# Peterande/SAST

Hardware: AMD Instinct MI355X
Metric: frames/sec (B=4) SAST backbone fwd+bwd, 1Mpx 640x360 (higher is better)
Workload: dtype f32; 1 GPU; 1Mpx 640x360 (padded 384x640) full SAST backbone + PAFPN, fwd+bwd + AdamW, B=4/GPU, binary events (rand>0.5), random-init, AMP=0.0002; global_batch=4, seq_len=1, parallelism=dp1, hipgraph=True, library=sast_amd/libsast_hip.so, product_library=True, segmented_backward_overlap=False, deferred_weight_gradients=False, backward_cuts=3, dw_discard_TIMING_PROBE_gradients_invalid=False, collective_ranks=1, collective_ranks_verified=1, gradient_bytes_per_rank=67663616, sync_batchnorm=False, event_dtype=int32, grads_finite=True

## Files before the change

### sast_amd/csrc/gemm.cuh

```cuda
#pragma once
#include <type_traits>
#include <hip/hip_ext.h>
#include "common.cuh"
#include "../../include/sast_hip.h"

#if defined(SAST_TL_ENABLE) && !defined(SAST_TL)
static __device__ unsigned long long sast_tl_buf[8 * 8192];
#define SAST_TL(k)                                                                                          \
  do {                                                                                                      \
    const unsigned bid_ = blockIdx.x;                                                                       \
    if (threadIdx.x == 0 && bid_ < 8192) sast_tl_buf[bid_ * 8 + (k)] = wall_clock64();                      \
    if (threadIdx.x == 0 && bid_ < 8192 && (k) == 0) sast_tl_buf[bid_ * 8 + 7] = __smid();                 \
  } while (0)
#define SAST_TL_JOB(j) do { if (threadIdx.x == 0 && blockIdx.x < 8192) sast_tl_buf[blockIdx.x * 8 + 6] = (j); } while (0)
#endif
#ifndef SAST_TL
#define SAST_TL(k)
#endif
#ifndef SAST_TL_JOB
#define SAST_TL_JOB(j)
#endif
#ifndef SAST_TLF
#define SAST_TLF_DECL
#define SAST_TLF(k)
// ... 118 lines not shown
template <class L, class = void> struct LoaderExactBf16 : std::false_type {};
template <class L> struct LoaderExactBf16<L, std::void_t<decltype(L::EXACT_BF16)>> : std::bool_constant<L::EXACT_BF16> {};
template <class L, class = void> struct LoaderExactAlways : std::false_type {};
template <class L> struct LoaderExactAlways<L, std::void_t<decltype(L::EXACT_BF16_ALWAYS)>> : std::bool_constant<L::EXACT_BF16_ALWAYS> {};
template <class EP, class = void> struct EpHasStats : std::false_type {};
template <class EP> struct EpHasStats<EP, std::void_t<decltype(EP::COLSTATS)>> : std::bool_constant<EP::COLSTATS> {};

using buf_rsrc = __amdgpu_buffer_rsrc_t;
constexpr unsigned BUF_INVALID = 0x80000000u;
constexpr unsigned BUF_MAX_BYTES = 0x80000000u;
__device__ __forceinline__ buf_rsrc make_buf(const void* p, unsigned bytes) {
  const unsigned long long a = reinterpret_cast<unsigned long long>(p);
  const unsigned lo = __builtin_amdgcn_readfirstlane((unsigned)a), hi = __builtin_amdgcn_readfirstlane((unsigned)(a >> 32));
  return __builtin_amdgcn_make_buffer_rsrc(reinterpret_cast<void*>(((unsigned long long)hi << 32) | lo), 0,
                                           __builtin_amdgcn_readfirstlane(bytes), 0x00020000);
}
__device__ __forceinline__ float4 ldb(buf_rsrc d, unsigned off) {
  return __builtin_bit_cast(float4, __builtin_amdgcn_raw_buffer_load_b128(d, off, 0, 0));
}
__device__ __forceinline__ float ldb1(buf_rsrc d, unsigned off) {
  return __uint_as_float(__builtin_amdgcn_raw_buffer_load_b32(d, off, 0, 0));
}
struct BufDesc { buf_rsrc d; };
template <class L, class = void> struct LoaderBuffered : std::false_type {};
template <class L> struct LoaderBuffered<L, std::void_t<decltype(L::BUFFERED)>> : std::bool_constant<L::BUFFERED> {};
struct NoDesc {};
template <class L> __device__ __forceinline__ auto loader_desc(const L& l, int Rl) {
  if constexpr (LoaderBuffered<L>::value) return l.desc(Rl); else return NoDesc{};
}
constexpr unsigned long long BUF_SPAN_LIMIT = 0x80000000ull;
constexpr int BUF_SPAN_SLACK_ROWS = 64;
template <class L> inline bool loader_span_ok(const L& l, int I, int G, int R) {
  if constexpr (LoaderBuffered<L>::value) return l.span_bytes(I, G, R) < BUF_SPAN_LIMIT; else return true;
}

template <class T, class L>
struct OperandPresplitWanted { static constexpr bool value = SAST_MFMA_SPLIT3 && !SAST_MFMA_BF16 && L::RC && (T::BK == 16 || T::BK == 32) && T::KS <= 4 && T::G < 3; };
constexpr int PS_ROW_FLOATS = 3 * 16 / 2;
__device__ __forceinline__ constexpr int ps_chunk_swizzle(int row) { return (row >> 3) & 1; }
constexpr int PS_MAX_FLOATS = 20480;
template <class T, class L, int W>
struct OperandPresplitIC {
  static constexpr bool value = SAST_MFMA_SPLIT3 && !SAST_MFMA_BF16 && !L::RC && (T::BK == 16 || T::BK == 32) && T::KS <= 4 && T::G < 3 &&
                                (W == 32 || W == 64 || W == 128);
};
template <int W> __device__ __forceinline__ constexpr int psi_swizzle(int k) { return W == 64 ? ((k >> 1) & 1) << 3 : W == 128 ? (k & 3) << 3 : 0; }
// ... 152 lines not shown
    for (int it = 0; it < A_PER; ++it)
      if (A_SLOTS % NT == 0 || tid + it * NT < A_SLOTS) {
        const float4 v = la.finish(ra[set][it], aa[set][it], oa[set][it]);
        if constexpr (SPLIT && !LA::RC) {
          if (do_colsum) { csacc[it].x += v.x; csacc[it].y += v.y; csacc[it].z += v.z; csacc[it].w += v.w; }
        }
        if constexpr (PSA && EA) store_hi(as + la_off[it], v);
        else if constexpr (PSA) store_split3(as + la_off[it], BM * 8, v);
        else st4(as + la_off[it], v);
      }
#pragma unroll
    for (int it = 0; it < B_PER; ++it)
      if (B_SLOTS % NT == 0 || tid + it * NT < B_SLOTS) {
        if constexpr (PSB && EB) store_hi(bs + lb_off[it], lb.finish(rb[set][it], ab[set][it], ob[set][it]));
        else if constexpr (PSB) store_split3(bs + lb_off[it], BN * 8, lb.finish(rb[set][it], ab[set][it], ob[set][it]));
        else st4(bs + lb_off[it], lb.finish(rb[set][it], ab[set][it], ob[set][it]));
      }
  };

  typename EP::Col ecol[T::TJ];
#pragma unroll
  for (int tj = 0; tj < T::TJ; ++tj) ecol[tj] = ep.col(min(j0 + (wn * T::TJ + tj) * 32 + (lane & 31), NJ - 1));
  constexpr bool EARLY_AUX = T::TM * T::TJ == 1;
  typename EP::Aux eaux[EARLY_AUX ? 16 : 1];

  f32x16 acc[T::TM][T::TN];
#pragma unroll
  for (int a = 0; a < T::TM; ++a)
#pragma unroll
    for (int b = 0; b < T::TN; ++b)
#pragma unroll
      for (int e = 0; e < 16; ++e) acc[a][b][e] = 0.f;
  float csum[T::TM];
#pragma unroll
  for (int a = 0; a < T::TM; ++a) csum[a] = 0.f;

  auto compute = [&](int buf, auto ex) {
    constexpr bool EA = decltype(ex)::value && XA, EB = decltype(ex)::value && XB;
    const float* as = As + buf * A_STAGE;
    const float* bs = Bs + buf * B_STAGE;
    const int l31 = lane & 31, hf = lane >> 5;
    if constexpr (SAST_MFMA_SPLIT3 && !SAST_MFMA_BF16 && PSA && PSB) {
#pragma unroll
      for (int u = 0; u < BK / 16; ++u) {
        Split3 sa[T::TM], sb[T::TN];
#pragma unroll
// ... 238 lines not shown
#pragma unroll
      for (int a = 0; a < T::TM; ++a)
#pragma unroll
        for (int b = 0; b < T::TN; ++b)
#pragma unroll
          for (int e = 0; e < 16; ++e) acc[a][b][e] += src[((a * T::TN + b) * 16 + e) * 64];
    }
  }

  if (SPLIT && LA::RC && do_colsum) {
#pragma unroll
    for (int t = 0; t < T::TM; ++t) {
      const float s = csum[t] + __shfl_xor(csum[t], 32, 64);
      const int m = m0 + wm * T::WTM + t * 32 + (lane & 31);
      if (lane < 32 && m < Meff) atomicAdd(colsum + m, s);
    }
  }

  SAST_TL(3);
  constexpr bool STATS = EpHasStats<EP>::value;
  float cs[T::TJ], cq[T::TJ];
#pragma unroll
  for (int tj = 0; tj < T::TJ; ++tj) { cs[tj] = 0.f; cq[tj] = 0.f; }
  auto emit = [&](auto inside) {
    constexpr bool INSIDE = decltype(inside)::value;
#pragma unroll
    for (int ta = 0; ta < T::TM; ++ta)
#pragma unroll
      for (int tj = 0; tj < T::TJ; ++tj) {
        const int j = j0 + (wn * T::TJ + tj) * 32 + (lane & 31);
        const int jc = INSIDE ? j : min(j, NJ - 1);
        const int mb = m0 + wm * T::WTM + ta * 32 + 4 * (lane >> 5);
        const typename EP::Col col = ecol[tj];
        typename EP::Aux aux[16];
#pragma unroll
        for (int reg = 0; reg < 16; ++reg) {
          if constexpr (EARLY_AUX) aux[reg] = eaux[reg];
          else aux[reg] = ep.pre(INSIDE ? mb + (reg & 3) + 8 * (reg >> 2) : min(mb + (reg & 3) + 8 * (reg >> 2), Meff - 1), jc);
        }
#pragma unroll
        for (int reg = 0; reg < 16; ++reg) {
          const int m = mb + (reg & 3) + 8 * (reg >> 2);
          if (INSIDE || (m < Meff && j < NJ)) {
            float v[G];
#pragma unroll
            for (int g = 0; g < G; ++g) v[g] = acc[ta][tj * G + g][reg];
            ep.post(m, j, v, col, aux[reg]);
            if constexpr (STATS) ep.stat(v[0], col, aux[reg], cs[tj], cq[tj]);
          }
        }
      }
  };
  if (m0 + BM <= Meff && j0 + BJ <= NJ) emit(std::true_type{});
  else emit(std::false_type{});
  if constexpr (STATS) {
#pragma unroll
    for (int tj = 0; tj < T::TJ; ++tj) {
      const float s = cs[tj] + __shfl_xor(cs[tj], 32, 64), q = cq[tj] + __shfl_xor(cq[tj], 32, 64);
      const int j = j0 + (wn * T::TJ + tj) * 32 + (lane & 31);
      if (lane < 32 && j < NJ) ep.flush(((m0 / BM) * T::WAVES_M + wm) % BN_STAT_COPIES, j, NJ, s, q);
    }
  }
  SAST_TL(4);
}

template <class T, class LA, class LB, class EP, bool SPLIT>
__global__ __launch_bounds__(T::NT, T::MINW) void gemm_kernel(LA la, LB lb, EP ep, int M, int NJ, int R,
                                                              const int* __restrict__ dM, const int* __restrict__ dR,
                                                              float* __restrict__ colsum, int nsplit, int xcd_remap) {
  __shared__ __attribute__((aligned(16))) float smem[GemmSmem<T, LA, LB>::FLOATS];
  kernarg_warm<(int)(sizeof(LA) + sizeof(LB) + sizeof(EP) + 3 * sizeof(int) + 3 * sizeof(void*) + 2 * sizeof(int))>();
  int nmain = gridDim.x;
  if constexpr (EpHasSide<EP>::value) {
    nmain -= ep.side_blocks;
    if ((int)blockIdx.x >= nmain) { ep.side(blockIdx.x - nmain); return; }
  }
  gemm_body<T, LA, LB, EP, SPLIT>(la, lb, ep, M, NJ, R, dM, dR, colsum, nsplit, xcd_remap, blockIdx.x, nmain, smem);
// ... 37 lines not shown
  static double get(const L& l) { return l.src_bytes(); }
};
void prof_kernel_events_ex(const char* tag, double flops, double bytes, hipStream_t st, hipEvent_t* e0, hipEvent_t* e1);
void prof_sum_k(const int* Kw, int W, hipStream_t st, double* sum_k, double* sum_k2);
bool prof_enabled();
void prof_flops_credit(double flops);
bool xcd_remap_enabled();
void prof_scope(const char* name, int c, int m, hipStream_t st, bool begin);
struct ProfScope {
  const char* n; int c, m; hipStream_t st; bool on;
  ProfScope(const char* n_, int c_, int m_, hipStream_t s_) : n(n_), c(c_), m(m_), st(s_), on(prof_enabled()) { if (on) prof_scope(n, c, m, st, true); }
  ~ProfScope() { if (on) prof_scope(n, c, m, st, false); }
};

template <class T, class LA, class LB>
inline bool gemm_span_ok(const LA& la, const LB& lb, int M, int NJ, int R) {
  return loader_span_ok(la, M, 1, R) && loader_span_ok(lb, NJ, T::G, R);
}

template <class T, class LA, class LB, class EP>
inline int launch_gemm(const LA& la, const LB& lb, const EP& ep, int M, int NJ, int R, const int* dM,
                       const int* dR, hipStream_t st) {
  if (M <= 0 || NJ <= 0 || R <= 0) return SAST_OK;
  if (!gemm_span_ok<T>(la, lb, M, NJ, R)) return SAST_EINVAL;
  const int nb = ((M + T::BM - 1) / T::BM) * ((NJ + T::BJ - 1) / T::BJ);
  const int remap = xcd_remap_enabled() && nb >= 16;
  const int grid = remap ? (nb + 7) / 8 * 8 : nb;
  if (prof_enabled()) {
    hipEvent_t e0, e1;
    prof_kernel_events(__PRETTY_FUNCTION__, T::G, M, NJ, R, dM, dR, st, &e0, &e1, LoaderSrcBytes<LA>::get(la), LoaderSrcBytes<LB>::get(lb));
    SAST_EXT_LAUNCH((gemm_kernel<T, LA, LB, EP, false>), dim3(grid + ep_side_blocks(ep)), dim3(T::NT), 0, st, e0, e1, 0, la, lb, ep, M, NJ,
                          R, dM, dR, (float*)nullptr, 1, remap);
  } else {
    SAST_LAUNCH((gemm_kernel<T, LA, LB, EP, false>), dim3(grid + ep_side_blocks(ep)), dim3(T::NT), 0, st, la, lb, ep, M, NJ, R, dM, dR,
                       (float*)nullptr, 1, remap);
  }
  SAST_CHECK_LAUNCH();
  return SAST_OK;
}

template <class T, class LA, class LB, class EP>
inline int launch_gemm_split(const LA& la, const LB& lb, const EP& ep, int M, int NJ, int R, const int* dR,
                             int splits, float* colsum, hipStream_t st) {
  if (M <= 0 || NJ <= 0 || R <= 0) return SAST_OK;
  if (colsum != nullptr && LA::RC && GemmSmem<T, LA, LB>::PSA) return SAST_EINVAL;
  if (!gemm_span_ok<T>(la, lb, M, NJ, R)) return SAST_EINVAL;
  const int nb = ((M + T::BM - 1) / T::BM) * ((NJ + T::BJ - 1) / T::BJ);
  if (splits < 1) splits = 1;
  const int remap = xcd_remap_enabled() && nb * splits >= 16;
  const int grid = remap ? (nb * splits + 7) / 8 * 8 : nb * splits;
  if (prof_enabled()) {
    hipEvent_t e0, e1;
    prof_kernel_events(__PRETTY_FUNCTION__, T::G, M, NJ, R, nullptr, dR, st, &e0, &e1, LoaderSrcBytes<LA>::get(la), LoaderSrcBytes<LB>::get(lb));
    SAST_EXT_LAUNCH((gemm_kernel<T, LA, LB, EP, true>), dim3(grid), dim3(T::NT), 0, st, e0, e1, 0, la, lb, ep, M, NJ, R,
                          (const int*)nullptr, dR, colsum, splits, remap);
  } else {
    SAST_LAUNCH((gemm_kernel<T, LA, LB, EP, true>), dim3(grid), dim3(T::NT), 0, st, la, lb, ep, M, NJ, R,
                       (const int*)nullptr, dR, colsum, splits, remap);
  }
  SAST_CHECK_LAUNCH();
  return SAST_OK;
}

inline int gemm_grid(int ntile, int nsplit, int& remap) {
  const int n = ntile * nsplit;
  remap = xcd_remap_enabled() && n >= 16;
  return remap ? (n + 7) / 8 * 8 : n;
}
void prof_kernel_events2(const char* tag, double flops_static, int G1, int M1, int NJ1, int R1, const int* dM1, const int* dR1, int G2,
                         int M2, int NJ2, int R2, const int* dM2, const int* dR2, hipStream_t st, hipEvent_t* e0, hipEvent_t* e1,
                         double a1_cap = -1.0, double b1_cap = -1.0, double a2_cap = -1.0, double b2_cap = -1.0);

template <class TS, class LA1, class LB1, class EP1, class TP, class LA2, class LB2, class EP2>
inline int launch_gemm_dual(const LA1& la1, const LB1& lb1, const EP1& ep1, int M1, int NJ1, int R1, const int* dR1, int splits,
                            float* colsum, const LA2& la2, const LB2& lb2, const EP2& ep2, int M2, int NJ2, int R2, const int* dM2,
                            hipStream_t st) {
  using J1 = GemmJob<TS, LA1, LB1, EP1, true>;
  using J2 = GemmJob<TP, LA2, LB2, EP2, false>;
  if (colsum != nullptr && LA1::RC && GemmSmem<TS, LA1, LB1>::PSA) return SAST_EINVAL;
  if (!gemm_span_ok<TS>(la1, lb1, M1, NJ1, R1) || !gemm_span_ok<TP>(la2, lb2, M2, NJ2, R2)) return SAST_EINVAL;
  if (splits < 1) splits = 1;
  const int nt1 = ((M1 + TS::BM - 1) / TS::BM) * ((NJ1 + TS::BJ - 1) / TS::BJ);
  const int nt2 = ((M2 + TP::BM - 1) / TP::BM) * ((NJ2 + TP::BJ - 1) / TP::BJ);
  int r1, r2;
  int n1 = gemm_grid(nt1, splits, r1);
  const int n2 = gemm_grid(nt2, 1, r2);
  if (r2 && (n1 & 7)) n1 = (n1 + 7) / 8 * 8;
  const J1 a{la1, lb1, ep1, M1, NJ1, R1, nullptr, dR1, colsum, splits, r1};
  const J2 b{la2, lb2, ep2, M2, NJ2, R2, dM2, nullptr, nullptr, 1, r2};
  constexpr int NTHREADS = TS::NT > TP::NT ? TS::NT : TP::NT;
  if (prof_enabled()) {
    hipEvent_t e0, e1;
    prof_kernel_events2(__PRETTY_FUNCTION__, 0.0, TS::G, M1, NJ1, R1, nullptr, dR1, TP::G, M2, NJ2, R2, dM2, nullptr, st, &e0, &e1,
                        LoaderSrcBytes<LA1>::get(la1), LoaderSrcBytes<LB1>::get(lb1), LoaderSrcBytes<LA2>::get(la2), LoaderSrcBytes<LB2>::get(lb2));
    SAST_EXT_LAUNCH((gemm_dual_kernel<J1, J2>), dim3(n1 + n2 + ep_side_blocks(ep2)), dim3(NTHREADS), 0, st, e0, e1, 0, a, b, n1);
  } else {
    SAST_LAUNCH((gemm_dual_kernel<J1, J2>), dim3(n1 + n2 + ep_side_blocks(ep2)), dim3(NTHREADS), 0, st, a, b, n1);
  }
  SAST_CHECK_LAUNCH();
  return SAST_OK;
}

using TileBig   = Tile<128, 128, 2, 2, 1>;
// ... 501 lines not shown
    return c;
  }
  __device__ __forceinline__ int reduce_len(int m0) const { return k.slots(m0 / k.Mc) * Cout; }
  __device__ __forceinline__ void load(const Desc& d, const Ctx& c, int r0, int off, int Rl, int, float4& v, float& aux, bool& ok) const {
    const int r = r0 + off, rr = min(r, Rl - 1);
    const int slot = (int)__umulhi((unsigned)rr, cout_mul), co = rr - slot * Cout;
    const int kh = (c.kh >> (4 * slot)) & 15, kw = (c.kw >> (4 * slot)) & 15;
    const bool empty = kh == 15 || kw == 15;
    ok = (r < Rl) & !empty;
    v = ldb(d.d, ok ? c.col + 4u * (unsigned)((co * taps + (empty ? 0 : kh * KW + kw)) * Cin) : BUF_INVALID);
    aux = 0.f;
  }
  SAST_DEFAULT_FINISH
};

inline int pow2_shift(int v) {
  int s = 0;
  while ((1 << s) < v) ++s;
  return (1 << s) == v ? s : -1;
}

struct EpNone {};
struct EpStore {
  float* c; int ldc; const float* bias;
  struct Col { float b; };
  using Aux = EpNone;
  __device__ __forceinline__ Col col(int j) const { return Col{bias ? bias[j] : 0.f}; }
  __device__ __forceinline__ Aux pre(int, int) const { return Aux{}; }
  __device__ __forceinline__ void post(int m, int j, const float (&v)[1], const Col& k, const Aux&) const {
    c[(size_t)m * ldc + j] = v[0] + k.b;
  }
};
struct EpStoreStats {
  static constexpr bool COLSTATS = true;
  float* c; int ldc; double* sums;
  using Col = EpNone; using Aux = EpNone;
  __device__ __forceinline__ Col col(int) const { return Col{}; }
  __device__ __forceinline__ Aux pre(int, int) const { return Aux{}; }
  __device__ __forceinline__ void post(int m, int j, const float (&v)[1], const Col&, const Aux&) const { c[(size_t)m * ldc + j] = v[0]; }
  __device__ __forceinline__ void stat(float v, const Col&, const Aux&, float& a, float& b) const { a += v; b += v * v; }
  __device__ __forceinline__ void flush(int copy, int j, int NJ, float s, float q) const {
    double* sp = sums + (size_t)copy * 2 * NJ;
    atomicAdd(sp + j, (double)s); atomicAdd(sp + NJ + j, (double)q);
  }
};

struct BnProducer {
  const float* x;
  const float* stats;
  const float* gamma; const float* beta;
  float* sums;
  int C;
};
struct BnCol { float mu, rs, g, b; };
__device__ __forceinline__ BnCol bn_col(const BnProducer& p, int j) { return BnCol{p.stats[j], p.stats[p.C + j], p.gamma[j], p.beta[j]}; }
__device__ __forceinline__ void bn_stat(float dy, float x, const BnCol& k, float& a, float& b) {
  const float xh = (x - k.mu) * k.rs;
  const float z = xh * k.g + k.b, sg = sigmoid_hw(z);
  const float dz = dy * sg * (1.f + z * (1.f - sg));
  a += dz; b += dz * xh;
}
struct EpStoreBnRed {
  static constexpr bool COLSTATS = true;
  float* c; int ldc; BnProducer p;
  using Col = BnCol;
  struct Aux { float x; };
  __device__ __forceinline__ Col col(int j) const { return bn_col(p, j); }
  __device__ __forceinline__ Aux pre(int m, int j) const { return Aux{p.x[(size_t)m * p.C + j]}; }
  __device__ __forceinline__ void post(int m, int j, const float (&v)[1], const Col&, const Aux&) const { c[(size_t)m * ldc + j] = v[0]; }
  __device__ __forceinline__ void stat(float v, const Col& k, const Aux& x, float& a, float& b) const { bn_stat(v, x.x, k, a, b); }
  __device__ __forceinline__ void flush(int copy, int j, int, float s, float q) const {
    float* sp = p.sums + (size_t)copy * 2 * p.C;
    atomicAdd(sp + j, s); atomicAdd(sp + p.C + j, q);
  }
};
struct EpStoreAdd {
  float* c; int ldc; const float* add; int ldadd;
  using Col = EpNone;
  struct Aux { float a; };
  __device__ __forceinline__ Col col(int) const { return Col{}; }
  __device__ __forceinline__ Aux pre(int m, int j) const { return Aux{add[(size_t)m * ldadd + j]}; }
  __device__ __forceinline__ void post(int m, int j, const float (&v)[1], const Col&, const Aux& x) const {
    c[(size_t)m * ldc + j] = v[0] + x.a;
  }
};
struct EpStoreStats2 {
  static constexpr bool COLSTATS = true;
  float* c1; float* c2; int C; double* sums1; double* sums2;
  using Col = EpNone; using Aux = EpNone;
  __device__ __forceinline__ Col col(int) const { return Col{}; }
  __device__ __forceinline__ Aux pre(int, int) const { return Aux{}; }
  __device__ __forceinline__ void post(int m, int j, const float (&v)[1], const Col&, const Aux&) const {
    if (j < C) c1[(size_t)m * C + j] = v[0];
    else c2[(size_t)m * C + (j - C)] = v[0];
  }
  __device__ __forceinline__ void stat(float v, const Col&, const Aux&, float& a, float& b) const { a += v; b += v * v; }
  __device__ __forceinline__ void flush(int copy, int j, int, float s, float q) const {
    double* sp = (j < C ? sums1 : sums2) + (size_t)copy * 2 * C;
    const int jj = j < C ? j : j - C;
    atomicAdd(sp + jj, (double)s); atomicAdd(sp + C + jj, (double)q);
  }
};
struct EpAtomic2 {
  float* c1; float* c2; int ldc; int M1;
  using Col = EpNone; using Aux = EpNone;
  __device__ __forceinline__ Col col(int) const { return Col{}; }
  __device__ __forceinline__ Aux pre(int, int) const { return Aux{}; }
  __device__ __forceinline__ void post(int m, int j, const float (&v)[1], const Col&, const Aux&) const {
    atomicAdd((m < M1 ? c1 + (size_t)m * ldc : c2 + (size_t)(m - M1) * ldc) + j, v[0]);
  }
};
struct EpAtomic {
  float* c; int ldc;
  using Col = EpNone; using Aux = EpNone;
  __device__ __forceinline__ Col col(int) const { return Col{}; }
  __device__ __forceinline__ Aux pre(int, int) const { return Aux{}; }
  __device__ __forceinline__ void post(int m, int j, const float (&v)[1], const Col&, const Aux&) const {
    atomicAdd(c + (size_t)m * ldc + j, v[0]);
  }
};

struct EpStoreClass {
  float* c; int ldc; int H, W; ConvDxClasses k;
  using Col = EpNone;
  struct Aux { int p; };
  __device__ __forceinline__ Col col(int) const { return Col{}; }
  __device__ __forceinline__ Aux pre(int m, int) const {
    const int cls = fast_div(m, k.Mc, k.mc_mul), ic = m - cls * k.Mc;
    const int t = fast_div(ic, k.Wc, k.wc_mul), xx = ic - t * k.Wc, b = fast_div(t, k.Hc, k.hc_mul), yy = t - b * k.Hc;
    const int q = 3 - cls;
    return Aux{(b * H + 2 * yy + (q >> 1)) * W + 2 * xx + (q & 1)};
  }
  __device__ __forceinline__ void post(int, int j, const float (&v)[1], const Col&, const Aux& a) const {
    c[(size_t)a.p * ldc + j] = v[0];
  }
};

struct EpSplit2BnRed {
  static constexpr bool COLSTATS = true;
  float* a; float* b; int C1, C2; BnProducer pa, pb;
  using Col = BnCol;
  struct Aux { float x; };
  __device__ __forceinline__ Col col(int j) const {
    if (j < C1) return pa.x ? bn_col(pa, j) : BnCol{0.f, 0.f, 0.f, 0.f};
    return pb.x ? bn_col(pb, j - C1) : BnCol{0.f, 0.f, 0.f, 0.f};
  }
  __device__ __forceinline__ Aux pre(int m, int j) const {
    if (j < C1) return Aux{pa.x ? pa.x[(size_t)m * C1 + j] : 0.f};
    return Aux{pb.x ? pb.x[(size_t)m * C2 + (j - C1)] : 0.f};
  }
  __device__ __forceinline__ void post(int m, int j, const float (&v)[1], const Col&, const Aux&) const {
    if (j < C1) a[(size_t)m * C1 + j] = v[0];
    else if (b) b[(size_t)m * C2 + (j - C1)] = v[0];
  }
  __device__ __forceinline__ void stat(float v, const Col& k, const Aux& x, float& s, float& q) const { bn_stat(v, x.x, k, s, q); }
  __device__ __forceinline__ void flush(int copy, int j, int, float s, float q) const {
    if (j < C1) {
      if (pa.x) { float* sp = pa.sums + (size_t)copy * 2 * C1; atomicAdd(sp + j, s); atomicAdd(sp + C1 + j, q); }
    } else if (pb.x) {
      float* sp = pb.sums + (size_t)copy * 2 * C2; atomicAdd(sp + (j - C1), s); atomicAdd(sp + C2 + (j - C1), q);
    }
  }
};

struct EpSplit2 {
  float* a; float* b; int C1, C2;
  using Col = EpNone; using Aux = EpNone;
  __device__ __forceinline__ Col col(int) const { return Col{}; }
  __device__ __forceinline__ Aux pre(int, int) const { return Aux{}; }
  __device__ __forceinline__ void post(int m, int j, const float (&v)[1], const Col&, const Aux&) const {
    if (j < C1) a[(size_t)m * C1 + j] = v[0];
    else if (b) b[(size_t)m * C2 + (j - C1)] = v[0];
  }
};

}
```

### sast_amd/csrc/gemm_kloop.inc

```
#pragma unroll
  for (int u = 0; u < PF; ++u) gload(tile_of(u), u);
  lstore(0, 0, ex);
  group_sync();
  SAST_TL(1);
  int i = 0;
  SAST_TLF_DECL
  for (; i + PF <= n_it; i += PF) {
#pragma unroll
    for (int u = 0; u < PF; ++u) {
      gload(tile_of(i + u + PF), u);
      SAST_PHASE_FENCE();
      SAST_TLF(0);
      compute(u & 1, ex);
      SAST_TLF(1);
      SAST_TLF_WAIT_OLDER(A_PER + B_PER);
      lstore((u + 1) & 1, (u + 1) % PF, ex);
      SAST_TLF(2);
      group_sync();
      SAST_TLF(3);
      SAST_TLF_COUNT();
    }
  }
  SAST_TLF_FLUSH();
  if constexpr (EARLY_AUX) {
    const int jc = min(j0 + wn * 32 + (lane & 31), NJ - 1), mb = m0 + wm * T::WTM + 4 * (lane >> 5);
#pragma unroll
    for (int reg = 0; reg < 16; ++reg) eaux[reg] = ep.pre(min(mb + (reg & 3) + 8 * (reg >> 2), Meff - 1), jc);
  }
  {
    const int rem = n_it - i;
#pragma unroll
    for (int u = 0; u < PF - 1; ++u) {
      if (u < rem) {
        compute(u & 1, ex);
        lstore((u + 1) & 1, (u + 1) % PF, ex);
        group_sync();
      }
    }
  }
```

### sast_amd/csrc/k_block.hip

```cpp
#include <cstdlib>
#include "gemm_dispatch.cuh"
#include "kernels.h"

using namespace sast;

namespace {

constexpr int ATTN_MAX_T = 256;

struct EpBiasRelu {
  float* c; int ldc; const float* bias;
  struct Col { float b; };
  using Aux = EpNone;
  __device__ __forceinline__ Col col(int j) const { return Col{bias[j]}; }
  __device__ __forceinline__ Aux pre(int, int) const { return Aux{}; }
  __device__ __forceinline__ void post(int m, int j, const float (&v)[1], const Col& k, const Aux&) const {
    c[(size_t)m * ldc + j] = fmaxf(v[0] + k.b, 0.f);
  }
};
struct EpBiasReluCtl : EpBiasRelu {
  static constexpr bool SIDE = true;
  ControlsJob k; int side_blocks;
  __device__ __forceinline__ void side(int sb) const { if (threadIdx.x < 256) controls_fwd_elem(k, sb * 256 + threadIdx.x); }
};
struct EpStoreAddCtl : EpStoreAdd {
  static constexpr bool SIDE = true;
  ControlsJob k; int side_blocks;
  __device__ __forceinline__ void side(int sb) const { if (threadIdx.x < 256) controls_bwd_elem(k, sb * 256 + threadIdx.x); }
};
template <bool RS>
struct EpResidualLST {
  float* y; const float* res; const float* bias; const float* gamma; int C; const float* rs;
  struct Col { float b, g; };
  struct Aux { float r, d; };
  __device__ __forceinline__ Col col(int j) const { return Col{bias[j], gamma ? gamma[j] : 1.f}; }
  __device__ __forceinline__ Aux pre(int m, int j) const { return Aux{res[(size_t)m * C + j], RS ? rs[m] : 1.f}; }
  __device__ __forceinline__ void post(int m, int j, const float (&v)[1], const Col& k, const Aux& x) const {
    if constexpr (RS) y[(size_t)m * C + j] = x.r + (k.g * (v[0] + k.b)) * x.d;
    else y[(size_t)m * C + j] = x.r + k.g * (v[0] + k.b);
  }
};
template <bool RS>
struct EpResidualLSScatterT {
  float* out; const float* res; const float* bias; const float* gamma; const int* row_tok; int C; const float* rs;
  struct Col { float b, g; };
  struct Aux { float r, d; int row; };
  __device__ __forceinline__ Col col(int j) const { return Col{bias[j], gamma ? gamma[j] : 1.f}; }
  __device__ __forceinline__ Aux pre(int m, int j) const { return Aux{res[(size_t)m * C + j], RS ? rs[m] : 1.f, row_tok[m]}; }
  __device__ __forceinline__ void post(int, int j, const float (&v)[1], const Col& k, const Aux& x) const {
    if constexpr (RS) out[(size_t)x.row * C + j] = x.r + (k.g * (v[0] + k.b)) * x.d;
    else out[(size_t)x.row * C + j] = x.r + k.g * (v[0] + k.b);
  }
};
constexpr int PRELU_SLOTS = 1024;
__global__ void __launch_bounds__(PRELU_SLOTS) prelu_slope_finish_kernel(const float* __restrict__ slots, float* __restrict__ d) {
  __shared__ float s[PRELU_SLOTS];
  s[threadIdx.x] = slots[threadIdx.x];
  __syncthreads();
  for (int o = PRELU_SLOTS / 2; o; o >>= 1) {
    if ((int)threadIdx.x < o) s[threadIdx.x] += s[threadIdx.x + o];
    __syncthreads();
  }
  if (threadIdx.x == 0) d[0] += s[0];
}
template <bool ANY>
struct EpGluT {
  float* ug; float* h; const float* bias; int inner; int act;
  const float* drop;
  const float* act_w;
  struct Col { float bu, bg, a; };
  using Aux = EpNone;
  __device__ __forceinline__ Col col(int j) const { return Col{bias[j], bias[inner + j], (ANY && act_w) ? act_w[0] : 0.0f}; }
  __device__ __forceinline__ Aux pre(int, int) const { return Aux{}; }
  __device__ __forceinline__ void post(int m, int j, const float (&v)[2], const Col& k, const Aux&) const {
    const float u = v[0] + k.bu, g = v[1] + k.bg;
    float* ugm = ug + (size_t)m * 2 * inner;
    ugm[j] = u;
    (ugm + inner)[j] = g;
    if constexpr (ANY) h[(size_t)m * inner + j] = (u * glu_act(g, act, k.a)) * (drop ? drop[(size_t)m * inner + j] : 1.f);
    else h[(size_t)m * inner + j] = u * gelu_erf(g);
  }
};
template <bool ANY>
struct EpDGluT {
  const float* ug; float* dug; int inner; int act;
  const float* drop;
  const float* act_w;
  float* slope_slots;
  struct Col { float a; };
  struct Aux { float u, g; };
  __device__ __forceinline__ Col col(int) const { return Col{(ANY && act_w) ? act_w[0] : 0.0f}; }
  __device__ __forceinline__ Aux pre(int m, int j) const { return Aux{ug[(size_t)m * 2 * inner + j], ug[(size_t)m * 2 * inner + inner + j]}; }
  __device__ __forceinline__ void post(int m, int j, const float (&v)[1], const Col& k, const Aux& x) const {
    if constexpr (ANY) {
      const float dh = drop ? v[0] * drop[(size_t)m * inner + j] : v[0];
      dug[(size_t)m * 2 * inner + j] = dh * glu_act(x.g, act, k.a);
      dug[(size_t)m * 2 * inner + inner + j] = dh * x.u * glu_act_grad(x.g, act, k.a);
      if (slope_slots && x.g < 0.0f) atomicAdd(slope_slots + (((size_t)m * inner + j) & (PRELU_SLOTS - 1)), dh * x.u * x.g);
    } else {
      dug[(size_t)m * 2 * inner + j] = v[0] * gelu_erf(x.g);
      dug[(size_t)m * 2 * inner + inner + j] = v[0] * x.u * gelu_erf_grad(x.g);
    }
  }
};
struct EpAddGather {
  float* c; int ldc; const float* src; const int* idx; int lds;
  using Col = EpNone;
  struct Aux { float a; };
  __device__ __forceinline__ Col col(int) const { return Col{}; }
  __device__ __forceinline__ Aux pre(int m, int j) const { return Aux{src[(size_t)idx[m] * lds + j]}; }
  __device__ __forceinline__ void post(int m, int j, const float (&v)[1], const Col&, const Aux& x) const {
    c[(size_t)m * ldc + j] = v[0] + x.a;
  }
};
struct EpLstm {
  const float* bias; const float* c0; float* h1; float* c1; float* gates; int C;
  const float* drop;
  struct Col { float bf, bi, bo, bg; };
  struct Aux { float c, d; };
  __device__ __forceinline__ Col col(int j) const { return Col{bias[j], bias[C + j], bias[2 * C + j], bias[3 * C + j]}; }
  __device__ __forceinline__ Aux pre(int m, int j) const { return Aux{c0 ? c0[(size_t)m * C + j] : 0.f, drop ? drop[(size_t)m * C + j] : 1.f}; }
  __device__ __forceinline__ void post(int m, int j, const float (&v)[4], const Col& k, const Aux& x) const {
    const float f = sigmoid_hw(v[0] + k.bf), i = sigmoid_hw(v[1] + k.bi);
    const float o = sigmoid_hw(v[2] + k.bo), g = tanh_hw(v[3] + k.bg);
    const float c = f * x.c + i * (g * x.d);
    c1[(size_t)m * C + j] = c;
    h1[(size_t)m * C + j] = o * tanh_hw(c);
    float* gp = gates + (size_t)m * 4 * C + j;
    gp[0] = f; gp[C] = i; gp[2 * C] = o; gp[3 * C] = g;
  }
};
struct EpLstm3 {
  const float* bias; float* h1; float* c1; float* gates; int C; const float* drop;
  struct Col { float bi, bo, bg; };
  struct Aux { float d; };
  __device__ __forceinline__ Col col(int j) const { return Col{bias[C + j], bias[2 * C + j], bias[3 * C + j]}; }
  __device__ __forceinline__ Aux pre(int m, int j) const { return Aux{drop ? drop[(size_t)m * C + j] : 1.f}; }
  __device__ __forceinline__ void post(int m, int j, const float (&v)[3], const Col& k, const Aux& x) const {
    const float i = sigmoid_hw(v[0] + k.bi), o = sigmoid_hw(v[1] + k.bo), g = tanh_hw(v[2] + k.bg);
    const float c = 0.f + i * (g * x.d);
    c1[(size_t)m * C + j] = c;
    h1[(size_t)m * C + j] = o * tanh_hw(c);
    float* gp = gates + (size_t)m * 4 * C + j;
    gp[C] = i; gp[2 * C] = o; gp[3 * C] = g;
  }
};
inline bool lstm_skip_f(const SastLstmArgs* a) { return !a->c0 && SAST_KNOB("SAST_LSTM_SKIP_DEAD_GATE", 1) != 0; }

template <bool SKIPF>
__global__ __launch_bounds__(256) void lstm_bwd_pointwise_kernel(const float* __restrict__ gates, const float* __restrict__ c0,
                                                                 const float* __restrict__ c1, const float* __restrict__ dh1,
                                                                 const float* __restrict__ dh1b, const float* __restrict__ dc1,
                                                                 float* __restrict__ dmix,
                                                                 float* __restrict__ dc0, size_t n, int C, unsigned c_mul,
                                                                 const float* __restrict__ drop) {
  const size_t e = (size_t)blockIdx.x * 256 + threadIdx.x;
  if (e >= n) return;
  const size_t m = fast_div((int)e, C, c_mul); const int j = (int)(e - m * C);
  const float* gp = gates + m * 4 * C + j;
  const float f = SKIPF ? 0.f : gp[0], i = gp[C], o = gp[2 * C], g = gp[3 * C];
  const float tc = tanh_hw(c1[e]);
  const float dh = dh1[e] + (dh1b ? dh1b[e] : 0.f);
  const float dc = (dc1 ? dc1[e] : 0.f) + dh * o * (1.f - tc * tc);
  const float cp = (!SKIPF && c0) ? c0[e] : 0.f;
  float* dp = dmix + m * 4 * C + j;
  if constexpr (!SKIPF) dp[0] = dc * cp * f * (1.f - f);
  const float d = drop ? drop[e] : 1.f;
// ... 390 lines not shown
```

Before: 888.5 frames/s.

## Use buffer-resource stores and loads in GEMM epilogues with hardware OOB masking

Adds a buffered epilogue path in which each epilogue builds AMDGPU buffer descriptors for its output and aux tensors and does every store and aux load through raw buffer ops. Offsets are 32-bit with wave-uniform bases, and out-of-range rows and columns are dropped by the descriptor bound or an invalid offset instead of per-element branches and clamping. This aims to cut 64-bit address arithmetic and branch overhead in the epilogue. The cost is span checks that reject tensors above 2GB and extra logic for split-output epilogues where a tile straddles the boundary between the two outputs.

New measurement: 895.0 frames/s (median of 6 runs). About the same (+0.7%).

```diff
diff --git a/sast_amd/csrc/gemm.cuh b/sast_amd/csrc/gemm.cuh
--- a/sast_amd/csrc/gemm.cuh
+++ b/sast_amd/csrc/gemm.cuh
@@ -164,6 +164,34 @@
   return __uint_as_float(__builtin_amdgcn_raw_buffer_load_b32(d, off, 0, 0));
 }
 struct BufDesc { buf_rsrc d; };
+__device__ __forceinline__ buf_rsrc out_buf(const void* p, int Meff, int ld) {
+  return make_buf(p, p ? 4u * (unsigned)Meff * (unsigned)ld : 0u);
+}
+__device__ __forceinline__ void stb(buf_rsrc d, unsigned off, float v) {
+  __builtin_amdgcn_raw_buffer_store_b32(__float_as_uint(v), d, off, 0, 0);
+}
+struct EpAt {
+  int m, j;
+  unsigned lane_col;
+  unsigned lane_rows;
+  int mu;
+  int jt;
+  __device__ __forceinline__ unsigned at(int ld, int dj = 0) const {
+    return (lane_col + 4u * (lane_rows * (unsigned)ld + (unsigned)dj)) + 4u * (unsigned)(mu * ld);
+  }
+};
+struct EpSide { bool right, straddle; };
+__device__ __forceinline__ EpSide ep_side(const EpAt& e, int C1) { return EpSide{e.jt + 32 > C1, e.jt < C1 && e.jt + 32 > C1}; }
+__device__ __forceinline__ EpAt ep_mask(EpAt e, bool keep) { e.lane_col = keep ? e.lane_col : BUF_INVALID; return e; }
+template <class EP, class = void> struct EpBuffered : std::false_type {};
+template <class EP> struct EpBuffered<EP, std::void_t<decltype(EP::BUFFERED)>> : std::bool_constant<EP::BUFFERED> {};
+constexpr int EP_SPAN_SLACK_ROWS = 128;
+inline bool ep_span(int M, int ld, int cols) {
+  return 4ull * ((unsigned long long)(M + EP_SPAN_SLACK_ROWS) * (unsigned long long)ld + (unsigned long long)cols) < 0x80000000ull;
+}
+template <class EP> inline bool ep_span_ok(const EP& ep, int M, int NJ) {
+  if constexpr (EpBuffered<EP>::value) return ep.span_ok(M, NJ); else return true;
+}
 template <class L, class = void> struct LoaderBuffered : std::false_type {};
 template <class L> struct LoaderBuffered<L, std::void_t<decltype(L::BUFFERED)>> : std::bool_constant<L::BUFFERED> {};
 struct NoDesc {};
@@ -362,6 +390,14 @@
 #pragma unroll
   for (int tj = 0; tj < T::TJ; ++tj) ecol[tj] = ep.col(min(j0 + (wn * T::TJ + tj) * 32 + (lane & 31), NJ - 1));
   constexpr bool EARLY_AUX = T::TM * T::TJ == 1;
+  struct EpBase { int mu0, jt0; };
+  auto ep_base = [&]() { return EpBase{__builtin_amdgcn_readfirstlane(m0 + wm * T::WTM), __builtin_amdgcn_readfirstlane(j0 + wn * T::TJ * 32)}; };
+  auto ep_at = [&](const EpBase& eb, int ta, int tj, int reg) {
+    const int j = j0 + (wn * T::TJ + tj) * 32 + (lane & 31);
+    const int mu = eb.mu0 + ta * 32 + (reg & 3) + 8 * (reg >> 2);
+    const unsigned lr = 4u * (unsigned)(lane >> 5);
+    return EpAt{mu + (int)lr, j, j < NJ ? 4u * (unsigned)j : BUF_INVALID, lr, mu, eb.jt0 + tj * 32};
+  };
   typename EP::Aux eaux[EARLY_AUX ? 16 : 1];
 
   f32x16 acc[T::TM][T::TN];
@@ -646,7 +682,7 @@
   float cs[T::TJ], cq[T::TJ];
 #pragma unroll
   for (int tj = 0; tj < T::TJ; ++tj) { cs[tj] = 0.f; cq[tj] = 0.f; }
-  auto emit = [&](auto inside) {
+  auto emit = [&](auto inside, const auto& epx) {
     constexpr bool INSIDE = decltype(inside)::value;
 #pragma unroll
     for (int ta = 0; ta < T::TM; ++ta)
@@ -660,7 +696,7 @@
 #pragma unroll
         for (int reg = 0; reg < 16; ++reg) {
           if constexpr (EARLY_AUX) aux[reg] = eaux[reg];
-          else aux[reg] = ep.pre(INSIDE ? mb + (reg & 3) + 8 * (reg >> 2) : min(mb + (reg & 3) + 8 * (reg >> 2), Meff - 1), jc);
+          else aux[reg] = epx.pre(INSIDE ? mb + (reg & 3) + 8 * (reg >> 2) : min(mb + (reg & 3) + 8 * (reg >> 2), Meff - 1), jc);
         }
 #pragma unroll
         for (int reg = 0; reg < 16; ++reg) {
@@ -669,14 +705,39 @@
             float v[G];
 #pragma unroll
             for (int g = 0; g < G; ++g) v[g] = acc[ta][tj * G + g][reg];
-            ep.post(m, j, v, col, aux[reg]);
-            if constexpr (STATS) ep.stat(v[0], col, aux[reg], cs[tj], cq[tj]);
+            epx.post(m, j, v, col, aux[reg]);
+            if constexpr (STATS) epx.stat(v[0], col, aux[reg], cs[tj], cq[tj]);
           }
         }
       }
   };
-  if (m0 + BM <= Meff && j0 + BJ <= NJ) emit(std::true_type{});
-  else emit(std::false_type{});
+  if constexpr (EpBuffered<EP>::value) {
+    const auto edesc = ep.desc(Meff);
+    const EpBase eb = ep_base();
+#pragma unroll
+    for (int ta = 0; ta < T::TM; ++ta)
+#pragma unroll
+      for (int tj = 0; tj < T::TJ; ++tj) {
+        const typename EP::Col col = ecol[tj];
+        typename EP::Aux aux[16];
+#pragma unroll
+        for (int reg = 0; reg < 16; ++reg) {
+          if constexpr (EARLY_AUX) aux[reg] = eaux[reg];
+          else aux[reg] = ep.pre(edesc, ep_at(eb, ta, tj, reg));
+        }
+#pragma unroll
+        for (int reg = 0; reg < 16; ++reg) {
+          float v[G];
+#pragma unroll
+          for (int g = 0; g < G; ++g) v[g] = acc[ta][tj * G + g][reg];
+          ep.post(edesc, ep_at(eb, ta, tj, reg), v, col, aux[reg]);
+          if constexpr (STATS) ep.stat(v[0], col, aux[reg], cs[tj], cq[tj]);
+        }
+      }
+  } else {
+    if (m0 + BM <= Meff && j0 + BJ <= NJ) emit(std::true_type{}, ep);
+    else emit(std::false_type{}, ep);
+  }
   if constexpr (STATS) {
 #pragma unroll
     for (int tj = 0; tj < T::TJ; ++tj) {
@@ -760,7 +821,7 @@
 inline int launch_gemm(const LA& la, const LB& lb, const EP& ep, int M, int NJ, int R, const int* dM,
                        const int* dR, hipStream_t st) {
   if (M <= 0 || NJ <= 0 || R <= 0) return SAST_OK;
-  if (!gemm_span_ok<T>(la, lb, M, NJ, R)) return SAST_EINVAL;
+  if (!gemm_span_ok<T>(la, lb, M, NJ, R) || !ep_span_ok(ep, M, NJ)) return SAST_EINVAL;
   const int nb = ((M + T::BM - 1) / T::BM) * ((NJ + T::BJ - 1) / T::BJ);
   const int remap = xcd_remap_enabled() && nb >= 16;
   const int grid = remap ? (nb + 7) / 8 * 8 : nb;
@@ -782,7 +843,7 @@
                              int splits, float* colsum, hipStream_t st) {
   if (M <= 0 || NJ <= 0 || R <= 0) return SAST_OK;
   if (colsum != nullptr && LA::RC && GemmSmem<T, LA, LB>::PSA) return SAST_EINVAL;
-  if (!gemm_span_ok<T>(la, lb, M, NJ, R)) return SAST_EINVAL;
+  if (!gemm_span_ok<T>(la, lb, M, NJ, R) || !ep_span_ok(ep, M, NJ)) return SAST_EINVAL;
   const int nb = ((M + T::BM - 1) / T::BM) * ((NJ + T::BJ - 1) / T::BJ);
   if (splits < 1) splits = 1;
   const int remap = xcd_remap_enabled() && nb * splits >= 16;
@@ -817,6 +878,7 @@
   using J2 = GemmJob<TP, LA2, LB2, EP2, false>;
   if (colsum != nullptr && LA1::RC && GemmSmem<TS, LA1, LB1>::PSA) return SAST_EINVAL;
   if (!gemm_span_ok<TS>(la1, lb1, M1, NJ1, R1) || !gemm_span_ok<TP>(la2, lb2, M2, NJ2, R2)) return SAST_EINVAL;
+  if (!ep_span_ok(ep1, M1, NJ1) || !ep_span_ok(ep2, M2, NJ2)) return SAST_EINVAL;
   if (splits < 1) splits = 1;
   const int nt1 = ((M1 + TS::BM - 1) / TS::BM) * ((NJ1 + TS::BJ - 1) / TS::BJ);
   const int nt2 = ((M2 + TP::BM - 1) / TP::BM) * ((NJ2 + TP::BJ - 1) / TP::BJ);
@@ -1364,22 +1426,29 @@
 
 struct EpNone {};
 struct EpStore {
+  static constexpr bool BUFFERED = true;
   float* c; int ldc; const float* bias;
   struct Col { float b; };
   using Aux = EpNone;
+  struct Desc { buf_rsrc c; };
+  bool span_ok(int M, int NJ) const { return ep_span(M, ldc, NJ); }
+  __device__ __forceinline__ Desc desc(int Meff) const { return Desc{out_buf(c, Meff, ldc)}; }
   __device__ __forceinline__ Col col(int j) const { return Col{bias ? bias[j] : 0.f}; }
-  __device__ __forceinline__ Aux pre(int, int) const { return Aux{}; }
-  __device__ __forceinline__ void post(int m, int j, const float (&v)[1], const Col& k, const Aux&) const {
-    c[(size_t)m * ldc + j] = v[0] + k.b;
+  __device__ __forceinline__ Aux pre(const Desc&, const EpAt&) const { return Aux{}; }
+  __device__ __forceinline__ void post(const Desc& d, const EpAt& e, const float (&v)[1], const Col& k, const Aux&) const {
+    stb(d.c, e.at(ldc), v[0] + k.b);
   }
 };
 struct EpStoreStats {
-  static constexpr bool COLSTATS = true;
+  static constexpr bool COLSTATS = true, BUFFERED = true;
   float* c; int ldc; double* sums;
   using Col = EpNone; using Aux = EpNone;
+  struct Desc { buf_rsrc c; };
+  bool span_ok(int M, int NJ) const { return ep_span(M, ldc, NJ); }
+  __device__ __forceinline__ Desc desc(int Meff) const { return Desc{out_buf(c, Meff, ldc)}; }
   __device__ __forceinline__ Col col(int) const { return Col{}; }
-  __device__ __forceinline__ Aux pre(int, int) const { return Aux{}; }
-  __device__ __forceinline__ void post(int m, int j, const float (&v)[1], const Col&, const Aux&) const { c[(size_t)m * ldc + j] = v[0]; }
+  __device__ __forceinline__ Aux pre(const Desc&, const EpAt&) const { return Aux{}; }
+  __device__ __forceinline__ void post(const Desc& d, const EpAt& e, const float (&v)[1], const Col&, const Aux&) const { stb(d.c, e.at(ldc), v[0]); }
   __device__ __forceinline__ void stat(float v, const Col&, const Aux&, float& a, float& b) const { a += v; b += v * v; }
   __device__ __forceinline__ void flush(int copy, int j, int NJ, float s, float q) const {
     double* sp = sums + (size_t)copy * 2 * NJ;
@@ -1403,13 +1472,16 @@
   a += dz; b += dz * xh;
 }
 struct EpStoreBnRed {
-  static constexpr bool COLSTATS = true;
+  static constexpr bool COLSTATS = true, BUFFERED = true;
   float* c; int ldc; BnProducer p;
   using Col = BnCol;
   struct Aux { float x; };
+  struct Desc { buf_rsrc c, x; };
+  bool span_ok(int M, int NJ) const { return ep_span(M, ldc, NJ) && ep_span(M, p.C, NJ); }
+  __device__ __forceinline__ Desc desc(int Meff) const { return Desc{out_buf(c, Meff, ldc), out_buf(p.x, Meff, p.C)}; }
   __device__ __forceinline__ Col col(int j) const { return bn_col(p, j); }
-  __device__ __forceinline__ Aux pre(int m, int j) const { return Aux{p.x[(size_t)m * p.C + j]}; }
-  __device__ __forceinline__ void post(int m, int j, const float (&v)[1], const Col&, const Aux&) const { c[(size_t)m * ldc + j] = v[0]; }
+  __device__ __forceinline__ Aux pre(const Desc& d, const EpAt& e) const { return Aux{ldb1(d.x, e.at(p.C))}; }
+  __device__ __forceinline__ void post(const Desc& d, const EpAt& e, const float (&v)[1], const Col&, const Aux&) const { stb(d.c, e.at(ldc), v[0]); }
   __device__ __forceinline__ void stat(float v, const Col& k, const Aux& x, float& a, float& b) const { bn_stat(v, x.x, k, a, b); }
   __device__ __forceinline__ void flush(int copy, int j, int, float s, float q) const {
     float* sp = p.sums + (size_t)copy * 2 * p.C;
@@ -1417,24 +1489,32 @@
   }
 };
 struct EpStoreAdd {
+  static constexpr bool BUFFERED = true;
   float* c; int ldc; const float* add; int ldadd;
   using Col = EpNone;
   struct Aux { float a; };
+  struct Desc { buf_rsrc c, add; };
+  bool span_ok(int M, int NJ) const { return ep_span(M, ldc, NJ) && ep_span(M, ldadd, NJ); }
+  __device__ __forceinline__ Desc desc(int Meff) const { return Desc{out_buf(c, Meff, ldc), out_buf(add, Meff, ldadd)}; }
   __device__ __forceinline__ Col col(int) const { return Col{}; }
-  __device__ __forceinline__ Aux pre(int m, int j) const { return Aux{add[(size_t)m * ldadd + j]}; }
-  __device__ __forceinline__ void post(int m, int j, const float (&v)[1], const Col&, const Aux& x) const {
-    c[(size_t)m * ldc + j] = v[0] + x.a;
+  __device__ __forceinline__ Aux pre(const Desc& d, const EpAt& e) const { return Aux{ldb1(d.add, e.at(ldadd))}; }
+  __device__ __forceinline__ void post(const Desc& d, const EpAt& e, const float (&v)[1], const Col&, const Aux& x) const {
+    stb(d.c, e.at(ldc), v[0] + x.a);
   }
 };
 struct EpStoreStats2 {
-  static constexpr bool COLSTATS = true;
+  static constexpr bool COLSTATS = true, BUFFERED = true;
   float* c1; float* c2; int C; double* sums1; double* sums2;
   using Col = EpNone; using Aux = EpNone;
+  struct Desc { buf_rsrc c1, c2; };
+  bool span_ok(int M, int) const { return ep_span(M, C, C); }
+  __device__ __forceinline__ Desc desc(int Meff) const { return Desc{out_buf(c1, Meff, C), out_buf(c2, Meff, C)}; }
   __device__ __forceinline__ Col col(int) const { return Col{}; }
-  __device__ __forceinline__ Aux pre(int, int) const { return Aux{}; }
-  __device__ __forceinline__ void post(int m, int j, const float (&v)[1], const Col&, const Aux&) const {
-    if (j < C) c1[(size_t)m * C + j] = v[0];
-    else c2[(size_t)m * C + (j - C)] = v[0];
+  __device__ __forceinline__ Aux pre(const Desc&, const EpAt&) const { return Aux{}; }
+  __device__ __forceinline__ void post(const Desc& d, const EpAt& e, const float (&v)[1], const Col&, const Aux&) const {
+    const EpSide sd = ep_side(e, C);
+    stb(sd.right ? d.c2 : d.c1, ep_mask(e, !sd.right || e.j >= C).at(C, sd.right ? -C : 0), v[0]);
+    if (sd.straddle) stb(d.c1, ep_mask(e, e.j < C).at(C), v[0]);
   }
   __device__ __forceinline__ void stat(float v, const Col&, const Aux&, float& a, float& b) const { a += v; b += v * v; }
   __device__ __forceinline__ void flush(int copy, int j, int, float s, float q) const {
@@ -1479,21 +1559,29 @@
 };
 
 struct EpSplit2BnRed {
-  static constexpr bool COLSTATS = true;
+  static constexpr bool COLSTATS = true, BUFFERED = true;
   float* a; float* b; int C1, C2; BnProducer pa, pb;
   using Col = BnCol;
   struct Aux { float x; };
+  struct Desc { buf_rsrc a, b, xa, xb; };
+  bool span_ok(int M, int) const { return ep_span(M, C1, C1) && ep_span(M, C2, C1 + C2); }
+  __device__ __forceinline__ Desc desc(int Meff) const {
+    return Desc{out_buf(a, Meff, C1), out_buf(b, Meff, C2), out_buf(pa.x, Meff, C1), out_buf(pb.x, Meff, C2)};
+  }
   __device__ __forceinline__ Col col(int j) const {
     if (j < C1) return pa.x ? bn_col(pa, j) : BnCol{0.f, 0.f, 0.f, 0.f};
     return pb.x ? bn_col(pb, j - C1) : BnCol{0.f, 0.f, 0.f, 0.f};
   }
-  __device__ __forceinline__ Aux pre(int m, int j) const {
-    if (j < C1) return Aux{pa.x ? pa.x[(size_t)m * C1 + j] : 0.f};
-    return Aux{pb.x ? pb.x[(size_t)m * C2 + (j - C1)] : 0.f};
-  }
-  __device__ __forceinline__ void post(int m, int j, const float (&v)[1], const Col&, const Aux&) const {
-    if (j < C1) a[(size_t)m * C1 + j] = v[0];
-    else if (b) b[(size_t)m * C2 + (j - C1)] = v[0];
+  __device__ __forceinline__ Aux pre(const Desc& d, const EpAt& e) const {
+    const EpSide sd = ep_side(e, C1);
+    float x = ldb1(sd.right ? d.xb : d.xa, ep_mask(e, !sd.right || e.j >= C1).at(sd.right ? C2 : C1, sd.right ? -C1 : 0));
+    if (sd.straddle) { const float xl = ldb1(d.xa, ep_mask(e, e.j < C1).at(C1)); x = e.j < C1 ? xl : x; }
+    return Aux{x};
+  }
+  __device__ __forceinline__ void post(const Desc& d, const EpAt& e, const float (&v)[1], const Col&, const Aux&) const {
+    const EpSide sd = ep_side(e, C1);
+    stb(sd.right ? d.b : d.a, ep_mask(e, !sd.right || e.j >= C1).at(sd.right ? C2 : C1, sd.right ? -C1 : 0), v[0]);
+    if (sd.straddle) stb(d.a, ep_mask(e, e.j < C1).at(C1), v[0]);
   }
   __device__ __forceinline__ void stat(float v, const Col& k, const Aux& x, float& s, float& q) const { bn_stat(v, x.x, k, s, q); }
   __device__ __forceinline__ void flush(int copy, int j, int, float s, float q) const {
@@ -1506,14 +1594,19 @@
 };
 
 struct EpSplit2 {
+  static constexpr bool BUFFERED = true;
   float* a; float* b; int C1, C2;
   using Col = EpNone; using Aux = EpNone;
+  struct Desc { buf_rsrc a, b; };
+  bool span_ok(int M, int) const { return ep_span(M, C1, C1) && ep_span(M, C2, C1 + C2); }
+  __device__ __forceinline__ Desc desc(int Meff) const { return Desc{out_buf(a, Meff, C1), out_buf(b, Meff, C2)}; }
   __device__ __forceinline__ Col col(int) const { return Col{}; }
-  __device__ __forceinline__ Aux pre(int, int) const { return Aux{}; }
-  __device__ __forceinline__ void post(int m, int j, const float (&v)[1], const Col&, const Aux&) const {
-    if (j < C1) a[(size_t)m * C1 + j] = v[0];
-    else if (b) b[(size_t)m * C2 + (j - C1)] = v[0];
-  }
-};
-
-}
+  __device__ __forceinline__ Aux pre(const Desc&, const EpAt&) const { return Aux{}; }
+  __device__ __forceinline__ void post(const Desc& d, const EpAt& e, const float (&v)[1], const Col&, const Aux&) const {
+    const EpSide sd = ep_side(e, C1);
+    stb(sd.right ? d.b : d.a, ep_mask(e, !sd.right || e.j >= C1).at(sd.right ? C2 : C1, sd.right ? -C1 : 0), v[0]);
+    if (sd.straddle) stb(d.a, ep_mask(e, e.j < C1).at(C1), v[0]);
+  }
+};
+
+}
diff --git a/sast_amd/csrc/gemm_kloop.inc b/sast_amd/csrc/gemm_kloop.inc
--- a/sast_amd/csrc/gemm_kloop.inc
+++ b/sast_amd/csrc/gemm_kloop.inc
@@ -22,7 +22,12 @@
     }
   }
   SAST_TLF_FLUSH();
-  if constexpr (EARLY_AUX) {
+  if constexpr (EARLY_AUX && EpBuffered<EP>::value) {
+    const auto edesc_early = ep.desc(Meff);
+    const auto eb_early = ep_base();
+#pragma unroll
+    for (int reg = 0; reg < 16; ++reg) eaux[reg] = ep.pre(edesc_early, ep_at(eb_early, 0, 0, reg));
+  } else if constexpr (EARLY_AUX) {
     const int jc = min(j0 + wn * 32 + (lane & 31), NJ - 1), mb = m0 + wm * T::WTM + 4 * (lane >> 5);
 #pragma unroll
     for (int reg = 0; reg < 16; ++reg) eaux[reg] = ep.pre(min(mb + (reg & 3) + 8 * (reg >> 2), Meff - 1), jc);
diff --git a/sast_amd/csrc/k_block.hip b/sast_amd/csrc/k_block.hip
--- a/sast_amd/csrc/k_block.hip
+++ b/sast_amd/csrc/k_block.hip
@@ -9,13 +9,17 @@
 constexpr int ATTN_MAX_T = 256;
 
 struct EpBiasRelu {
+  static constexpr bool BUFFERED = true;
   float* c; int ldc; const float* bias;
   struct Col { float b; };
   using Aux = EpNone;
+  struct Desc { buf_rsrc c; };
+  bool span_ok(int M, int NJ) const { return ep_span(M, ldc, NJ); }
+  __device__ __forceinline__ Desc desc(int Meff) const { return Desc{out_buf(c, Meff, ldc)}; }
   __device__ __forceinline__ Col col(int j) const { return Col{bias[j]}; }
-  __device__ __forceinline__ Aux pre(int, int) const { return Aux{}; }
-  __device__ __forceinline__ void post(int m, int j, const float (&v)[1], const Col& k, const Aux&) const {
-    c[(size_t)m * ldc + j] = fmaxf(v[0] + k.b, 0.f);
+  __device__ __forceinline__ Aux pre(const Desc&, const EpAt&) const { return Aux{}; }
+  __device__ __forceinline__ void post(const Desc& d, const EpAt& e, const float (&v)[1], const Col& k, const Aux&) const {
+    stb(d.c, e.at(ldc), fmaxf(v[0] + k.b, 0.f));
   }
 };
 struct EpBiasReluCtl : EpBiasRelu {
@@ -30,9 +34,17 @@
 };
 template <bool RS>
 struct EpResidualLST {
+  static constexpr bool BUFFERED = !RS;
   float* y; const float* res; const float* bias; const float* gamma; int C; const float* rs;
   struct Col { float b, g; };
   struct Aux { float r, d; };
+  struct Desc { buf_rsrc y, res; };
+  bool span_ok(int M, int NJ) const { return ep_span(M, C, NJ); }
+  __device__ __forceinline__ Desc desc(int Meff) const { return Desc{out_buf(y, Meff, C), out_buf(res, Meff, C)}; }
+  __device__ __forceinline__ Aux pre(const Desc& d, const EpAt& e) const { return Aux{ldb1(d.res, e.at(C)), 1.f}; }
+  __device__ __forceinline__ void post(const Desc& d, const EpAt& e, const float (&v)[1], const Col& k, const Aux& x) const {
+    stb(d.y, e.at(C), x.r + k.g * (v[0] + k.b));
+  }
   __device__ __forceinline__ Col col(int j) const { return Col{bias[j], gamma ? gamma[j] : 1.f}; }
   __device__ __forceinline__ Aux pre(int m, int j) const { return Aux{res[(size_t)m * C + j], RS ? rs[m] : 1.f}; }
   __device__ __forceinline__ void post(int m, int j, const float (&v)[1], const Col& k, const Aux& x) const {
@@ -70,6 +82,17 @@
   const float* act_w;
   struct Col { float bu, bg, a; };
   using Aux = EpNone;
+  static constexpr bool BUFFERED = !ANY;
+  struct Desc { buf_rsrc ug, h; };
+  bool span_ok(int M, int NJ) const { return ep_span(M, 2 * inner, inner + NJ); }
+  __device__ __forceinline__ Desc desc(int Meff) const { return Desc{out_buf(ug, Meff, 2 * inner), out_buf(h, Meff, inner)}; }
+  __device__ __forceinline__ Aux pre(const Desc&, const EpAt&) const { return Aux{}; }
+  __device__ __forceinline__ void post(const Desc& d, const EpAt& e, const float (&v)[2], const Col& k, const Aux&) const {
+    const float u = v[0] + k.bu, g = v[1] + k.bg;
+    stb(d.ug, e.at(2 * inner), u);
+    stb(d.ug, e.at(2 * inner, inner), g);
+    stb(d.h, e.at(inner), u * gelu_erf(g));
+  }
   __device__ __forceinline__ Col col(int j) const { return Col{bias[j], bias[inner + j], (ANY && act_w) ? act_w[0] : 0.0f}; }
   __device__ __forceinline__ Aux pre(int, int) const { return Aux{}; }
   __device__ __forceinline__ void post(int m, int j, const float (&v)[2], const Col& k, const Aux&) const {
@@ -89,6 +112,17 @@
   float* slope_slots;
   struct Col { float a; };
   struct Aux { float u, g; };
+  static constexpr bool BUFFERED = !ANY;
+  struct Desc { buf_rsrc ug, dug; };
+  bool span_ok(int M, int NJ) const { return ep_span(M, 2 * inner, inner + NJ); }
+  __device__ __forceinline__ Desc desc(int Meff) const { return Desc{out_buf(ug, Meff, 2 * inner), out_buf(dug, Meff, 2 * inner)}; }
+  __device__ __forceinline__ Aux pre(const Desc& d, const EpAt& e) const {
+    return Aux{ldb1(d.ug, e.at(2 * inner)), ldb1(d.ug, e.at(2 * inner, inner))};
+  }
+  __device__ __forceinline__ void post(const Desc& d, const EpAt& e, const float (&v)[1], const Col&, const Aux& x) const {
+    stb(d.dug, e.at(2 * inner), v[0] * gelu_erf(x.g));
+    stb(d.dug, e.at(2 * inner, inner), v[0] * x.u * gelu_erf_grad(x.g));
+  }
   __device__ __forceinline__ Col col(int) const { return Col{(ANY && act_w) ? act_w[0] : 0.0f}; }
   __device__ __forceinline__ Aux pre(int m, int j) const { return Aux{ug[(size_t)m * 2 * inner + j], ug[(size_t)m * 2 * inner + inner + j]}; }
   __device__ __forceinline__ void post(int m, int j, const float (&v)[1], const Col& k, const Aux& x) const {
@@ -118,31 +152,48 @@
   const float* drop;
   struct Col { float bf, bi, bo, bg; };
   struct Aux { float c, d; };
+  static constexpr bool BUFFERED = true;
+  struct Desc { buf_rsrc c0, drop, h1, c1, gates; };
+  bool span_ok(int M, int NJ) const { return ep_span(M, 4 * C, 3 * C + NJ); }
+  __device__ __forceinline__ Desc desc(int Meff) const {
+    return Desc{out_buf(c0, Meff, C), out_buf(drop, Meff, C), out_buf(h1, Meff, C), out_buf(c1, Meff, C), out_buf(gates, Meff, 4 * C)};
+  }
   __device__ __forceinline__ Col col(int j) const { return Col{bias[j], bias[C + j], bias[2 * C + j], bias[3 * C + j]}; }
-  __device__ __forceinline__ Aux pre(int m, int j) const { return Aux{c0 ? c0[(size_t)m * C + j] : 0.f, drop ? drop[(size_t)m * C + j] : 1.f}; }
-  __device__ __forceinline__ void post(int m, int j, const float (&v)[4], const Col& k, const Aux& x) const {
+  __device__ __forceinline__ Aux pre(const Desc& d, const EpAt& e) const {
+    const float dv = ldb1(d.drop, e.at(C));
+    return Aux{ldb1(d.c0, e.at(C)), drop ? dv : 1.f};
+  }
+  __device__ __forceinline__ void post(const Desc& d, const EpAt& e, const float (&v)[4], const Col& k, const Aux& x) const {
     const float f = sigmoid_hw(v[0] + k.bf), i = sigmoid_hw(v[1] + k.bi);
     const float o = sigmoid_hw(v[2] + k.bo), g = tanh_hw(v[3] + k.bg);
     const float c = f * x.c + i * (g * x.d);
-    c1[(size_t)m * C + j] = c;
-    h1[(size_t)m * C + j] = o * tanh_hw(c);
-    float* gp = gates + (size_t)m * 4 * C + j;
-    gp[0] = f; gp[C] = i; gp[2 * C] = o; gp[3 * C] = g;
+    stb(d.c1, e.at(C), c);
+    stb(d.h1, e.at(C), o * tanh_hw(c));
+    stb(d.gates, e.at(4 * C), f); stb(d.gates, e.at(4 * C, C), i);
+    stb(d.gates, e.at(4 * C, 2 * C), o); stb(d.gates, e.at(4 * C, 3 * C), g);
   }
 };
 struct EpLstm3 {
   const float* bias; float* h1; float* c1; float* gates; int C; const float* drop;
   struct Col { float bi, bo, bg; };
   struct Aux { float d; };
+  static constexpr bool BUFFERED = true;
+  struct Desc { buf_rsrc drop, h1, c1, gates; };
+  bool span_ok(int M, int NJ) const { return ep_span(M, 4 * C, 3 * C + NJ); }
+  __device__ __forceinline__ Desc desc(int Meff) const {
+    return Desc{out_buf(drop, Meff, C), out_buf(h1, Meff, C), out_buf(c1, Meff, C), out_buf(gates, Meff, 4 * C)};
+  }
   __device__ __forceinline__ Col col(int j) const { return Col{bias[C + j], bias[2 * C + j], bias[3 * C + j]}; }
-  __device__ __forceinline__ Aux pre(int m, int j) const { return Aux{drop ? drop[(size_t)m * C + j] : 1.f}; }
-  __device__ __forceinline__ void post(int m, int j, const float (&v)[3], const Col& k, const Aux& x) const {
+  __device__ __forceinline__ Aux pre(const Desc& d, const EpAt& e) const {
+    const float dv = ldb1(d.drop, e.at(C));
+    return Aux{drop ? dv : 1.f};
+  }
+  __device__ __forceinline__ void post(const Desc& d, const EpAt& e, const float (&v)[3], const Col& k, const Aux& x) const {
     const float i = sigmoid_hw(v[0] + k.bi), o = sigmoid_hw(v[1] + k.bo), g = tanh_hw(v[2] + k.bg);
     const float c = 0.f + i * (g * x.d);
-    c1[(size_t)m * C + j] = c;
-    h1[(size_t)m * C + j] = o * tanh_hw(c);
-    float* gp = gates + (size_t)m * 4 * C + j;
-    gp[C] = i; gp[2 * C] = o; gp[3 * C] = g;
+    stb(d.c1, e.at(C), c);
+    stb(d.h1, e.at(C), o * tanh_hw(c));
+    stb(d.gates, e.at(4 * C, C), i); stb(d.gates, e.at(4 * C, 2 * C), o); stb(d.gates, e.at(4 * C, 3 * C), g);
   }
 };
 inline bool lstm_skip_f(const SastLstmArgs* a) { return !a->c0 && SAST_KNOB("SAST_LSTM_SKIP_DEAD_GATE", 1) != 0; }
```
